# yynil/RWKVTTS

Measured on AMD Instinct MI355X. Metric: audio-tokens/sec/GPU (train fwd+bwd) RWKV7-0.4B L=4096; 1->8 GPU scaling, higher is better.
Workload: dtype bf16; 1 GPU; RWKV7-0.4B Spark layout train step (fwd+bwd+AdamW), B=8/GPU L=4096, synthetic text+speech tokens, random init (BASELINE.json configs[1]); global_batch=8, seq_len=4096, parallelism=dp1, grad_allreduce=none

## Files before the change

### include/rwkv7_hip.h

```cpp
#ifndef RWKV7_HIP_H
#define RWKV7_HIP_H

#include <stddef.h>

#ifdef __cplusplus
extern "C" {
#endif

#define RWKV7_OK 0
#define RWKV7_EINVAL (-1)
#define RWKV7_ECHUNK (-2)
#define RWKV7_EHEAD  (-3)
#define RWKV7_ESHAPE (-4)

#define RWKV7_HEAD_SIZE 64
#define RWKV7_CHUNK_LEN 16

typedef void *rwkv7_stream_t;

const char *rwkv7_version(void);

int rwkv7_wkv_fwd_bf16(int B, int T, int H, const void *w, const void *q, const void *k, const void *v,
                       const void *a, const void *b, void *y, float *s, float *sa, rwkv7_stream_t stream);
int rwkv7_wkv_fwd_f32(int B, int T, int H, const void *w, const void *q, const void *k, const void *v,
// ... 145 lines not shown
                            int nblocks, rwkv7_stream_t stream);
int rwkv7_tmix_post_bwd_compact_bf16(long rows, int D, const void *dout, const void *y, const void *r, const void *k,
                                     const void *v, const void *g, const void *gn_w, const void *gn_b, const void *r_k,
                                     float eps, void *d_y, void *dt, void *d_g, float *hscal, float *dparams_partial,
                                     int nblocks, rwkv7_stream_t stream);
int rwkv7_tmix_post_bwd_compact_f32(long rows, int D, const void *dout, const void *y, const void *r, const void *k,
                                    const void *v, const void *g, const void *gn_w, const void *gn_b, const void *r_k,
                                    float eps, void *d_y, void *dt, void *d_g, float *hscal, float *dparams_partial,
                                    int nblocks, rwkv7_stream_t stream);

int rwkv7_relusq_fwd_bf16(long n, const void *x, void *y, rwkv7_stream_t stream);
int rwkv7_relusq_fwd_f32(long n, const void *x, void *y, rwkv7_stream_t stream);
int rwkv7_relusq_bwd_bf16(long n, const void *x, const void *dy, void *dx, rwkv7_stream_t stream);
int rwkv7_relusq_bwd_f32(long n, const void *x, const void *dy, void *dx, rwkv7_stream_t stream);
int rwkv7_relusq_bwd_s_bf16(long n, const void *s, const void *dy, void *dx, rwkv7_stream_t stream);
int rwkv7_relusq_bwd_s_f32(long n, const void *s, const void *dy, void *dx, rwkv7_stream_t stream);

#define RWKV7_CHUNK_T 32
#define RWKV7_Q15_REC (64 * 64 + 2 * 256)
int rwkv7_wkv_chunk_prep_bf16(int B, int T, int H, const void *w, const void *a, const void *b, float *tinv,
                              rwkv7_stream_t stream);
int rwkv7_wkv_chunk_prep_f32(int B, int T, int H, const void *w, const void *a, const void *b, float *tinv,
                             rwkv7_stream_t stream);
int rwkv7_wkv_chunk_fwd_bf16(int B, int T, int H, const void *w, const void *q, const void *k, const void *v,
                             const void *a, const void *b, const float *tinv, void *y, float *sa, void *hs,
                             rwkv7_stream_t stream);
int rwkv7_wkv_chunk_fwd_f32(int B, int T, int H, const void *w, const void *q, const void *k, const void *v,
                            const void *a, const void *b, const float *tinv, void *y, float *sa, void *hs,
                            rwkv7_stream_t stream);
int rwkv7_wkv_chunk_fwd_seq_bf16(int B, int T, int H, const void *w, const void *q, const void *k, const void *v,
                                 const void *a, const void *b, const float *tinv, void *y, float *sa, void *hs,
                                 const int *seq_chunk_off, int nseq, rwkv7_stream_t stream);
int rwkv7_wkv_chunk_fwd_seq_f32(int B, int T, int H, const void *w, const void *q, const void *k, const void *v,
                                const void *a, const void *b, const float *tinv, void *y, float *sa, void *hs,
                                const int *seq_chunk_off, int nseq, rwkv7_stream_t stream);
int rwkv7_wkv_chunk_bseq_bf16(int B, int T, int H, const void *w, const void *q, const void *a, const void *b, const void *dy,
                              const float *tinv, void *e_vk, float *z, const int *seq_chunk_off, int nseq, rwkv7_stream_t stream);
int rwkv7_wkv_chunk_bwd_out_z_bf16(int B, int T, int H, const void *w, const void *q, const void *k, const void *v,
                                   const void *a, const void *b, const void *dy, const void *hs, const float *sa,
                                   const float *z, const void *e_vk, void *dw, void *dq, void *dk, void *dv,
                                   void *da, void *db, rwkv7_stream_t stream);
int rwkv7_wkv_chunk_fwd_state_bf16(int B, int T, int H, const void *w, const void *q, const void *k, const void *v,
                                   const void *a, const void *b, const float *tinv, void *y, float *sa, void *hs,
                                   const float *h0, float *hT, rwkv7_stream_t stream);
int rwkv7_wkv_chunk_bseq_state_bf16(int B, int T, int H, const void *w, const void *q, const void *a, const void *b,
                                    const void *dy, const float *tinv, void *e_vk, float *z,
// ... 193 lines not shown
```

### rwkvtts_amd/csrc/capi.hip

```cpp
#include <hip/hip_runtime.h>
#include <math.h>

#include "../../include/rwkv7_hip.h"

namespace rwkv7 {
int wkv_fwd_bf16(int, int, int, const void *, const void *, const void *, const void *, const void *, const void *,
                 void *, float *, float *, float *, int, hipStream_t);
int wkv_fwd_f32(int, int, int, const void *, const void *, const void *, const void *, const void *, const void *,
                void *, float *, float *, float *, int, hipStream_t);
int wkv_bwd_bf16(int, int, int, const void *, const void *, const void *, const void *, const void *, const void *,
                 const void *, const float *, const float *, void *, void *, void *, void *, void *, void *,
                 hipStream_t);
int wkv_bwd_f32(int, int, int, const void *, const void *, const void *, const void *, const void *, const void *,
                const void *, const float *, const float *, void *, void *, void *, void *, void *, void *,
                hipStream_t);

int wkv_bwd_split_bf16(int, int, int, const void *, const void *, const void *, const void *, const void *, const void *,
                       const void *, const float *, const float *, void *const *, void *const *, void *const *, void *,
                       void *const *, void *const *, int, hipStream_t);
int wkv_bwd_split_f32(int, int, int, const void *, const void *, const void *, const void *, const void *, const void *,
                      const void *, const float *, const float *, void *const *, void *const *, void *const *, void *,
                      void *const *, void *const *, int, hipStream_t);
int chunk_prep_bf16(int, int, int, const void *, const void *, const void *, float *, hipStream_t);
int chunk_prep_f32(int, int, int, const void *, const void *, const void *, float *, hipStream_t);
int chunk_fwd_bf16(int, int, int, const void *, const void *, const void *, const void *, const void *, const void *,
                   const float *, void *, float *, void *, const int *, int, hipStream_t);
int chunk_fwd_f32(int, int, int, const void *, const void *, const void *, const void *, const void *, const void *,
                  const float *, void *, float *, void *, const int *, int, hipStream_t);
int chunk_debug_mma(const float *, const float *, float *, float *, hipStream_t);
int chunk_debug_tr16(const uint16_t *, const int *, uint16_t *, hipStream_t);
int gemv32_bf16(int, int, int, const void *, const void *, const void *, void *, hipStream_t);
int ce_fwd_bwd(long, int, long, void *, const long *, long, float, float *, float, hipStream_t);
int adamw_step(long, float *, const void *, float *, float *, void *, const uint8_t *, const float *, const float *, float, float, float, float,
               float, float, float, hipStream_t);
int lora32_bf16(int, int, int, int, int, const void *, const void *, const void *, const void *, void *, hipStream_t);
int chunk_bseq_bf16(int, int, int, const void *, const void *, const void *, const void *, const void *, const float *, void *,
                    float *, const int *, int, hipStream_t);
int chunk_bseq_state_seq_bf16(int, int, int, const void *, const void *, const void *, const void *, const void *, const float *,
                              void *, float *, const int *, int, const float *, float *, hipStream_t);
int chunk_fwd9_state_seq_bf16(int, int, int, const void *, const void *, const void *, const void *, const void *, const void *,
                              const float *, void *, float *, void *, const int *, int, const float *, float *, hipStream_t);
int gemm_nt4_bf16(int, int, int, const void *, const void *, void *, const void *, int, hipStream_t);
struct MixLoraDesc {
    int nb;
    int r[4], off[4];
    int act[4];
    const void *w1[4];
// ... 393 lines not shown
                                   rwkv7_stream_t stream) {                                                         \
        if (B <= 0 || T <= 0 || H <= 0 || any_null({w, a, b, tinv})) return RWKV7_EINVAL;                           \
        if (T % RWKV7_CHUNK_T != 0) return RWKV7_ECHUNK;                                                            \
        return rwkv7::chunk_prep_##SFX(B, T, H, w, a, b, tinv, (hipStream_t)stream);                                \
    }                                                                                                               \
    int rwkv7_wkv_chunk_fwd_##SFX(int B, int T, int H, const void *w, const void *q, const void *k, const void *v,  \
                                  const void *a, const void *b, const float *tinv, void *y, float *sa, void *hs,   \
                                  rwkv7_stream_t stream) {                                                          \
        if (B <= 0 || T <= 0 || H <= 0 || any_null({w, q, k, v, a, b, tinv, y})) return RWKV7_EINVAL;               \
        if ((sa == nullptr) != (hs == nullptr)) return RWKV7_EINVAL;                                                \
        if (T % RWKV7_CHUNK_T != 0) return RWKV7_ECHUNK;                                                            \
        return rwkv7::chunk_fwd_##SFX(B, T, H, w, q, k, v, a, b, tinv, y, sa, hs, nullptr, 0, (hipStream_t)stream); \
    }                                                                                                               \
    int rwkv7_wkv_chunk_fwd_seq_##SFX(int B, int T, int H, const void *w, const void *q, const void *k, const void *v, \
                                      const void *a, const void *b, const float *tinv, void *y, float *sa, void *hs, \
                                      const int *seq_chunk_off, int nseq, rwkv7_stream_t stream) {                  \
        if (B <= 0 || T <= 0 || H <= 0 || any_null({w, q, k, v, a, b, tinv, y})) return RWKV7_EINVAL;               \
        if ((sa == nullptr) != (hs == nullptr) || (seq_chunk_off != nullptr && nseq <= 0)) return RWKV7_EINVAL;    \
        if (T % RWKV7_CHUNK_T != 0) return RWKV7_ECHUNK;                                                            \
        return rwkv7::chunk_fwd_##SFX(B, T, H, w, q, k, v, a, b, tinv, y, sa, hs, seq_chunk_off, nseq, (hipStream_t)stream); \
    }
CHUNK_DEFINE(bf16)
CHUNK_DEFINE(f32)
int rwkv7_wkv_chunk_bseq_bf16(int B, int T, int H, const void *w, const void *q, const void *a, const void *b, const void *dy,
                              const float *tinv, void *e_vk, float *z, const int *seq_chunk_off, int nseq, rwkv7_stream_t stream) {
    if (B <= 0 || T <= 0 || H <= 0 || any_null({w, q, a, b, dy, (const void *)tinv, (const void *)e_vk})) return RWKV7_EINVAL;
    if (seq_chunk_off != nullptr && nseq <= 0) return RWKV7_EINVAL;
    if (T % 32 != 0) return RWKV7_ECHUNK;
    return rwkv7::chunk_bseq_bf16(B, T, H, w, q, a, b, dy, tinv, e_vk, z, seq_chunk_off, nseq, (hipStream_t)stream);
}
int rwkv7_wkv_chunk_fwd_state_seq_bf16(int B, int T, int H, const void *w, const void *q, const void *k, const void *v,
                                       const void *a, const void *b, const float *tinv, void *y, float *sa, void *hs,
                                       const int *seq_chunk_off, int nseq, const float *h0, float *hT, rwkv7_stream_t stream) {
    if (B <= 0 || T <= 0 || H <= 0 || any_null({w, q, k, v, a, b, (const void *)tinv, y})) return RWKV7_EINVAL;
    if ((sa == nullptr) != (hs == nullptr)) return RWKV7_EINVAL;
    if ((seq_chunk_off == nullptr) != (nseq <= 0)) return RWKV7_EINVAL;
    if (T % 32 != 0) return RWKV7_ECHUNK;
    return rwkv7::chunk_fwd9_state_seq_bf16(B, T, H, w, q, k, v, a, b, tinv, y, sa, hs, seq_chunk_off, nseq, h0, hT, (hipStream_t)stream);
}
int rwkv7_wkv_chunk_bseq_state_seq_bf16(int B, int T, int H, const void *w, const void *q, const void *a, const void *b,
                                        const void *dy, const float *tinv, void *e_vk, float *z, const int *seq_chunk_off, int nseq,
                                        const float *dhT, float *dh0, rwkv7_stream_t stream) {
    if (B <= 0 || T <= 0 || H <= 0 || any_null({w, q, a, b, dy, (const void *)tinv, (const void *)e_vk})) return RWKV7_EINVAL;
    if ((seq_chunk_off == nullptr) != (nseq <= 0)) return RWKV7_EINVAL;
    if (T % 32 != 0) return RWKV7_ECHUNK;
    return rwkv7::chunk_bseq_state_seq_bf16(B, T, H, w, q, a, b, dy, tinv, e_vk, z, seq_chunk_off, nseq, dhT, dh0, (hipStream_t)stream);
// ... 399 lines not shown
```

### rwkvtts_amd/csrc/elementwise.hip

```cpp
#include "ln_row.h"

namespace rwkv7 {

__device__ __forceinline__ float sigmoidf_(float x) { return 1.0f / (1.0f + __expf(-x)); }

template <typename T, int NMIX>
__global__ __launch_bounds__(kEwMaxThreads) void mix_fwd_kernel(int B, int T_, int D, const T *__restrict__ x, const T *__restrict__ x_prev,
                               const T *__restrict__ mask, const T *__restrict__ params, T *__restrict__ out) {
    const int c = threadIdx.x * 8;
    const long rows = (long)B * T_;
    float p[NMIX][8];
#pragma unroll
    for (int i = 0; i < NMIX; i++) V8<T>::ld(params + (long)i * D + c, p[i]);
    const bool has_mask = mask != nullptr;
    const T *const maskq = has_mask ? mask : params;
    for (long row = blockIdx.x; row < rows; row += gridDim.x) {
        const int t = (int)(row % T_);
        const long rp = row > 0 ? row - 1 : 0;
        Raw8<T> qc, qp;
        qc.load(x + row * D + c);
        qp.load(x + rp * D + c);
        const float mc0 = V8<T>::ld1(maskq + (has_mask ? row : 0)), mp0 = V8<T>::ld1(maskq + (has_mask ? rp : 0));
        float xc[8], xp[8];
        qc.get(xc);
        qp.get(xp);
        const float mc = has_mask ? mc0 : 1.f, mp = (has_mask ? mp0 : 1.f) * (t > 0 ? 1.f : 0.f);
#pragma unroll
// ... 93 lines not shown
            for (int i = 0; i < NMIX; i++) {
                float gc[8];
                A.g[i].get(gc);
#pragma unroll
                for (int j = 0; j < 8; j++) {
                    acc[j] = fmaf(gc[j], 1.f - p[i][j], acc[j]);
                    acc[j] = fmaf(gn[i][j], p[i][j], acc[j]);
                    dp[i][j] = fmaf(gc[j], xp[j] - xc[j], dp[i][j]);
                    gn[i][j] = gc[j] * first;
                }
            }
#pragma unroll
            for (int j = 0; j < 8; j++) {
                acc[j] *= m;
                xc[j] = xq[j];
            }
            V8<T>::st(dx + row * D + c, acc);
            A = Bn;
        }
    }
#pragma unroll
    for (int i = 0; i < NMIX; i++) V8<float>::st(dpart + ((long)blockIdx.x * NMIX + i) * D + c, dp[i]);
}

__device__ __forceinline__ float softplus_(float u) { return u > 20.f ? u : log1pf(__expf(u)); }

template <typename T>
__global__ __launch_bounds__(kEwMaxThreads) void tmix_prepare_fwd_kernel(long rows, int D, const T *__restrict__ w_pre, const T *__restrict__ k,
                                        const T *__restrict__ v, const T *__restrict__ a_pre,
                                        const T *__restrict__ v_pre, const T *__restrict__ v_first,
                                        const T *__restrict__ mask, const T *__restrict__ k_k,
                                        const T *__restrict__ k_a, T *__restrict__ w_out, T *__restrict__ k_out,
                                        T *__restrict__ v_out, T *__restrict__ a_out, T *__restrict__ b_out) {
    const int c = threadIdx.x * 8;
    float kk_p[8], ka_p[8];
    V8<T>::ld(k_k + c, kk_p);
    V8<T>::ld(k_a + c, ka_p);
    for (long row = blockIdx.x; row < rows; row += gridDim.x) {
        const long o = row * D + c;
        const float m = mask ? V8<T>::ld1(mask + row) : 1.f;
        float z[8], kx[8], vx[8], ap[8];
        V8<T>::ld(w_pre + o, z);
        V8<T>::ld(k + o, kx);
        V8<T>::ld(v + o, vx);
        V8<T>::ld(a_pre + o, ap);
        float wo[8], ko[8], vo[8], ao[8], bo[8], kkr[8];
        float ss = 0.f;
#pragma unroll
        for (int j = 0; j < 8; j++) {
            wo[j] = (-softplus_(-z[j]) - 0.5f) * m;
            kx[j] *= m;
            vx[j] *= m;
            kkr[j] = kx[j] * kk_p[j];
            ss = fmaf(kkr[j], kkr[j], ss);
        }
        if (v_pre) {
            float vp[8], vf[8];
            V8<T>::ld(v_pre + o, vp);
            V8<T>::ld(v_first + o, vf);
#pragma unroll
            for (int j = 0; j < 8; j++) vx[j] = fmaf(vf[j] - vx[j], sigmoidf_(vp[j]), vx[j]);
        }
        ss = sum8(ss);
        const float inv = m / fmaxf(sqrtf(ss), 1e-12f);
#pragma unroll
        for (int j = 0; j < 8; j++) {
            const float a = sigmoidf_(ap[j]);
            const float kk = kkr[j] * inv;
            ko[j] = kx[j] * fmaf(a - 1.f, ka_p[j], 1.f);
            vo[j] = vx[j] * m;
            ao[j] = -kk;
            bo[j] = kk * a;
        }
        V8<T>::st(w_out + o, wo);
        V8<T>::st(k_out + o, ko);
        V8<T>::st(v_out + o, vo);
        V8<T>::st(a_out + o, ao);
        V8<T>::st(b_out + o, bo);
    }
}

template <typename T>
struct PrepBwdExtra {
    const T *d_w_b, *d_k2_b, *d_k2_c, *d_v2_b, *d_a_b, *d_b_b;
    const T *d_r_a, *d_r_b, *d_r_c;
    T *d_r;
    const T *d_vfirst_in;
    const T *dt, *r, *r_k;
    const float *hscal;
};

template <typename T, bool MULTI>
__global__ __launch_bounds__(kEwMaxThreads) void tmix_prepare_bwd_kernel(long rows, int D, const T *__restrict__ w_pre, const T *__restrict__ k,
                                        const T *__restrict__ v, const T *__restrict__ a_pre,
                                        const T *__restrict__ v_pre, const T *__restrict__ v_first,
                                        const T *__restrict__ mask, const T *__restrict__ k_k,
// ... 1302 lines not shown
```

### rwkvtts_amd/csrc/ln_row.h

```cpp
#pragma once
#include "wkv7_common.h"

namespace rwkv7 {

constexpr int kEwMaxThreads = 512;

typedef __bf16 pkbf2_t __attribute__((ext_vector_type(2)));
typedef float pkf2_t __attribute__((ext_vector_type(2)));
__device__ __forceinline__ uint32_t pk_bf16(float a, float b) {
    const pkf2_t v = {a, b};
    return __builtin_bit_cast(uint32_t, __builtin_convertvector(v, pkbf2_t));
}

template <typename T>
struct V8;
template <>
struct V8<bf16_t> {
    static __device__ __forceinline__ void ld(const bf16_t *p, float (&f)[8]) {
        const uint4 r = *reinterpret_cast<const uint4 *>(p);
        f[0] = __uint_as_float(r.x << 16); f[1] = __uint_as_float(r.x & 0xffff0000u);
        f[2] = __uint_as_float(r.y << 16); f[3] = __uint_as_float(r.y & 0xffff0000u);
        f[4] = __uint_as_float(r.z << 16); f[5] = __uint_as_float(r.z & 0xffff0000u);
        f[6] = __uint_as_float(r.w << 16); f[7] = __uint_as_float(r.w & 0xffff0000u);
    }
    static __device__ __forceinline__ void st(bf16_t *p, const float (&f)[8]) {
        uint4 r;
        r.x = pk_bf16(f[0], f[1]);
        r.y = pk_bf16(f[2], f[3]);
        r.z = pk_bf16(f[4], f[5]);
        r.w = pk_bf16(f[6], f[7]);
        *reinterpret_cast<uint4 *>(p) = r;
    }
    static __device__ __forceinline__ float ld1(const bf16_t *p) { return bf2f(p->x); }
};
template <>
struct V8<float> {
    static __device__ __forceinline__ void ld(const float *p, float (&f)[8]) {
        const float4 a = *reinterpret_cast<const float4 *>(p), b = *reinterpret_cast<const float4 *>(p + 4);
        f[0] = a.x; f[1] = a.y; f[2] = a.z; f[3] = a.w; f[4] = b.x; f[5] = b.y; f[6] = b.z; f[7] = b.w;
    }
    static __device__ __forceinline__ void st(float *p, const float (&f)[8]) {
        *reinterpret_cast<float4 *>(p) = make_float4(f[0], f[1], f[2], f[3]);
        *reinterpret_cast<float4 *>(p + 4) = make_float4(f[4], f[5], f[6], f[7]);
    }
    static __device__ __forceinline__ float ld1(const float *p) { return *p; }
};

template <typename T>
struct Raw8;
template <>
struct Raw8<bf16_t> {
    uint4 r;
    __device__ __forceinline__ void load(const bf16_t *p) { r = *reinterpret_cast<const uint4 *>(p); }
    __device__ __forceinline__ void get(float (&f)[8]) const {
        f[0] = __uint_as_float(r.x << 16); f[1] = __uint_as_float(r.x & 0xffff0000u);
// ... 76 lines not shown
#pragma unroll
    for (int j = 0; j < 8; j++) s += v[j];
    block_sum2(s, dummy, red, ph, ng);
    ph ^= 2;
    mu = s * inv_d;
    float q = 0.f;
    dummy = 0.f;
#pragma unroll
    for (int j = 0; j < 8; j++) {
        v[j] -= mu;
        q = fmaf(v[j], v[j], q);
    }
    block_sum2(q, dummy, red, ph, ng);
    ph ^= 2;
    rs = rsqrtf(q * inv_d + eps);
    const float m = has_mask ? f.m : 1.f;
#pragma unroll
    for (int j = 0; j < 8; j++) hm[j] = round_to<T>(fmaf(v[j] * rs, gm[j], bt[j]));
    if (write && h_out) V8<T>::st(h_out + o, hm);
#pragma unroll
    for (int j = 0; j < 8; j++) hm[j] *= m;
}

}
```

### rwkvtts_amd/csrc/wkv7_chunk_fwd.hip

```cpp
#include "chunk_common.h"
#include "launch_attr.h"

namespace rwkv7 {

#ifdef WKV7C_TIMING
__device__ long long g_chunk_timing[4 * 16];
#define TSTAMP(i)                                                                  \
    do {                                                                           \
        const long long now_ = __builtin_readcyclecounter();                       \
        if (blockIdx.x == 0 && lane == 0) g_chunk_timing[wave * 16 + (i)] += now_ - tprev_; \
        tprev_ = now_;                                                             \
    } while (0)
#else
#define TSTAMP(i) do { } while (0)
#endif

template <typename T>
__device__ __forceinline__ float ld_scalar(const T *p);
template <>
__device__ __forceinline__ float ld_scalar<bf16_t>(const bf16_t *p) { return bf2f(p->x); }
template <>
__device__ __forceinline__ float ld_scalar<float>(const float *p) { return *p; }

template <typename T>
__global__ __launch_bounds__(64) __attribute__((amdgpu_waves_per_eu(4, 4))) void wkv7c_prep_kernel(int T_, int H, const T *__restrict__ w_, const T *__restrict__ a_,
                                                        const T *__restrict__ b_, float *__restrict__ tinv_) {
    constexpr int LD = kC + kPad;
    __shared__ __attribute__((aligned(16))) uint16_t planes[4 * kC * LD];
    uint16_t *ATh = planes, *ATl = planes + kC * LD, *BHh = planes + 2 * kC * LD, *BHl = planes + 3 * kC * LD;
    static_assert(2 * kC * LD * 2 >= kC * 2 * 16 * 4, "the back substitution's A^T copy must fit over the a~ planes");
    const int nc = T_ / kC;
    const int bh = blockIdx.x / nc, c = blockIdx.x - bh * nc;
    const int bb = bh / H, hh = bh - bb * H;
    const int lane = threadIdx.x;
    const int kc = lane & 31, th = lane >> 5;
    const long tstride = (long)H * kN;
    const long base = (((long)bb * T_ + (long)c * kC + 16 * th) * H + hh) * kN + kc;
    float wv[2][16], av_[2][16], bv_[2][16];
#pragma unroll
    for (int p = 0; p < 2; p++)
#pragma unroll
        for (int j = 0; j < 16; j++) {
            const long idx = base + 32 * p + j * tstride;
            wv[p][j] = ld_scalar<T>(w_ + idx);
            av_[p][j] = ld_scalar<T>(a_ + idx);
            bv_[p][j] = ld_scalar<T>(b_ + idx);
        }
    f32x16 acc = zero16();
#pragma unroll
    for (int p = 0; p < 2; p++) {
        float lw[16], tot = 0.f;
#pragma unroll
        for (int j = 0; j < 16; j++) {
            lw[j] = -fast_exp(wv[p][j]);
            tot += lw[j];
        }
        const float first = __shfl(tot, kc);
        float G = th ? first : 0.f;
        if (p == 1) __syncthreads();
#pragma unroll
        for (int j = 0; j < 16; j++) {
            const int t = 16 * th + j;
            const float at = av_[p][j] * fast_exp(G);
            G += lw[j];
            const float bh_ = bv_[p][j] * fast_exp(-G);
            split2(at, ATh[t * LD + kc], ATl[t * LD + kc]);
            split2(bh_, BHh[t * LD + kc], BHl[t * LD + kc]);
        }
        __syncthreads();
        mma_tile3<kC>(acc, BHh, BHl, LD, ATh, ATl, LD, lane);
// ... 342 lines not shown
    for (int i = lane; i < kC * kC; i += 64) DT[i] = bf2f(Oh[(i / kC) * LDC + i % kC]) + bf2f(Ol[(i / kC) * LDC + i % kC]);
}

typedef short v4s_t __attribute__((ext_vector_type(4)));
__global__ __launch_bounds__(64) void tr16_probe_kernel(const uint16_t *__restrict__ in, const int *__restrict__ addr,
                                                        uint16_t *__restrict__ out) {
    __shared__ __attribute__((aligned(16))) uint16_t sm[4096];
    for (int i = threadIdx.x; i < 4096; i += 64) sm[i] = in[i];
    __syncthreads();
    const int lane = threadIdx.x;
    const v4s_t r = __builtin_amdgcn_ds_read_tr16_b64_v4i16((v4s_t __attribute__((address_space(3))) *)(sm + addr[lane]));
#pragma unroll
    for (int j = 0; j < 4; j++) out[lane * 4 + j] = (uint16_t)r[j];
}
int chunk_debug_tr16(const uint16_t *in, const int *addr, uint16_t *out, hipStream_t st) {
    (void)hipGetLastError();
    hipLaunchKernelGGL(tr16_probe_kernel, dim3(1), dim3(64), 0, st, in, addr, out);
    return (int)hipGetLastError();
}

template <typename T>
static int launch_prep(int B, int T_, int H, const void *w, const void *a, const void *b, float *tinv, hipStream_t st) {
    (void)hipGetLastError();
    hipLaunchKernelGGL((wkv7c_prep_kernel<T>), dim3(B * H * (T_ / kC)), dim3(64), 0, st, T_, H, (const T *)w, (const T *)a,
                       (const T *)b, tinv);
    return (int)hipGetLastError();
}

template <typename T, bool SAVE>
static int launch_fwd_t(int B, int T_, int H, const void *w, const void *q, const void *k, const void *v, const void *a,
                        const void *b, const float *tinv, void *y, float *sa, void *hs, const int *seq_off, int nseq,
                        hipStream_t st) {
    static DynLdsOnce lds_once;
    if (hipError_t e = lds_once.ensure(reinterpret_cast<const void *>(&wkv7c_fwd_kernel<T, SAVE>), (int)FwdSmem::total<T>()); e != hipSuccess) return (int)e;
    (void)hipGetLastError();
    hipLaunchKernelGGL((wkv7c_fwd_kernel<T, SAVE>), dim3((seq_off ? nseq : B) * H * 2), dim3(256), FwdSmem::total<T>(), st, T_, H,
                       (const T *)w, (const T *)q, (const T *)k, (const T *)v, (const T *)a, (const T *)b, tinv, (T *)y, sa, (uint16_t *)hs, seq_off);
    return (int)hipGetLastError();
}

int chunk_prep_bf16(int B, int T_, int H, const void *w, const void *a, const void *b, float *tinv, hipStream_t st) {
    return launch_prep<bf16_t>(B, T_, H, w, a, b, tinv, st);
}
int chunk_prep_f32(int B, int T_, int H, const void *w, const void *a, const void *b, float *tinv, hipStream_t st) {
    return launch_prep<float>(B, T_, H, w, a, b, tinv, st);
}
int chunk_fwd9_bf16(int, int, int, const void *, const void *, const void *, const void *, const void *, const void *, const float *,
                    void *, float *, void *, const int *, int, hipStream_t);

int chunk_fwd_bf16(int B, int T_, int H, const void *w, const void *q, const void *k, const void *v, const void *a,
                   const void *b, const float *tinv, void *y, float *sa, void *hs, const int *seq_off, int nseq, hipStream_t st) {
    return chunk_fwd9_bf16(B, T_, H, w, q, k, v, a, b, tinv, y, sa, hs, seq_off, nseq, st);
}
#ifdef RWKV7_LAB
int chunk_fwd4_bf16(int B, int T_, int H, const void *w, const void *q, const void *k, const void *v, const void *a,
                    const void *b, const float *tinv, void *y, float *sa, void *hs, const int *seq_off, int nseq, hipStream_t st) {
    return (sa && hs) ? launch_fwd_t<bf16_t, true>(B, T_, H, w, q, k, v, a, b, tinv, y, sa, hs, seq_off, nseq, st)
                      : launch_fwd_t<bf16_t, false>(B, T_, H, w, q, k, v, a, b, tinv, y, nullptr, nullptr, seq_off, nseq, st);
}
#endif
int chunk_fwd_f32(int B, int T_, int H, const void *w, const void *q, const void *k, const void *v, const void *a,
                  const void *b, const float *tinv, void *y, float *sa, void *hs, const int *seq_off, int nseq, hipStream_t st) {
    return (sa && hs) ? launch_fwd_t<float, true>(B, T_, H, w, q, k, v, a, b, tinv, y, sa, hs, seq_off, nseq, st)
// ... 20 lines not shown
```

### rwkvtts_amd/fused.py

```python
import ctypes
import os

import torch

from . import _lib

_FWD_BLOCKS = 32768
_MIX_FWD_BLOCKS = 2048
_BWD_BLOCKS = 1024
_MIX_BWD_ROWS = 4
_MIX_BWD_BLOCKS = 1024


def _p(t):
    return None if t is None else ctypes.c_void_p(t.data_ptr())


def _stream(t):
    return ctypes.c_void_p(torch.cuda.current_stream(t.device).cuda_stream)


def _sfx(t):
    if not t.is_cuda:
        raise NotImplementedError("fused RWKV-7 stages run on the HIP device only (no CPU path)")
# ... 539 lines not shown
        y, r, k, v, g, gn_w, gn_b, r_k = ctx.saved_tensors
        B, T, D = y.shape
        rows = B * T
        nb = min(rows, _BWD_BLOCKS)
        dout = _c(dout)
        d_y, d_r, d_k, d_v, d_g = [torch.empty_like(y) for _ in range(5)]
        part = torch.empty(nb, 3, D, dtype=torch.float32, device=y.device)
        _call("tmix_post_bwd", y, ctypes.c_long(rows), D, _p(dout), _p(y), _p(r), _p(k), _p(v), _p(g), _p(gn_w), _p(gn_b), _p(r_k),
              ctypes.c_float(ctx.eps), _p(d_y), _p(d_r), _p(d_k), _p(d_v), _p(d_g), _p(part), nb)
        dp = _colsum(part, y.dtype)
        return d_y, d_r, d_k, d_v, d_g, dp[0], dp[1], dp[2], None


def tmix_post(y, r, k, v, g, gn_weight, gn_bias, r_k, H, eps):
    return _TmixPost.apply(y, r, k, v, g, gn_weight, gn_bias, r_k.reshape(-1), eps)


CHAIN_VFIRST_GRAD = True
CHUNKED_WKV_BWD = True
CHUNKED_WKV_FWD = True
VIA_REFERENCE_OP = False


class _TmixCore(torch.autograd.Function):

    @staticmethod
    def forward(ctx, r, w_pre, k, v, a_pre, g, v_pre, v_first, k_k, k_a, gn_w, gn_b, r_k, mask, H, eps, seq_start=None):
        from . import ops
        B, T, D = k.shape
        if T % ops.CHUNK_LEN != 0:
            raise ValueError(f"T={T} must be a multiple of {ops.CHUNK_LEN}")
        r, w_pre, k, v, a_pre, g = _c(r), _c(w_pre), _c(k), _c(v), _c(a_pre), _c(g)
        v_pre = None if v_pre is None else _c(v_pre)
        v_first = None if v_first is None else _c(v_first)
        k_k, k_a = _c(k_k.to(k.dtype)), _c(k_a.to(k.dtype))
        gn_w, gn_b, r_k = _c(gn_w.to(k.dtype)), _c(gn_b.to(k.dtype)), _c(r_k.reshape(-1).to(k.dtype))
        rows = B * T
        w, k2, v2, a_in, b_in = [torch.empty_like(k) for _ in range(5)]
        _call("tmix_prepare_fwd", k, ctypes.c_long(rows), D, _p(w_pre), _p(k), _p(v), _p(a_pre), _p(v_pre), _p(v_first),
              _p(mask), _p(k_k), _p(k_a), _p(w), _p(k2), _p(v2), _p(a_in), _p(b_in), min(rows, _FWD_BLOCKS))
        v4 = lambda t: t.view(B, T, H, 64)
        via_op = VIA_REFERENCE_OP and seq_start is None
        chunked = CHUNKED_WKV_FWD and CHUNKED_WKV_BWD and k.dtype == torch.bfloat16 and T % ops.CHUNK_T == 0 and not via_op
        if seq_start is not None and not chunked:
            raise ValueError("packed rows (seq_start) need the chunked WKV7 kernels: bf16 tensors, T % 32 == 0")
        if chunked:
            y4, tinv, sa, s = ops.wkv7_chunk_forward(v4(w), v4(r), v4(k2), v4(v2), v4(a_in), v4(b_in), seq_off=seq_start)
            y = y4.view(B, T, D)
        else:
            tinv = None
            y = torch.empty_like(k)
            s = torch.empty(B, H, T // ops.CHUNK_LEN, 64, 64, dtype=torch.float32, device=k.device)
            sa = torch.empty(B, T, H, 64, dtype=torch.float32, device=k.device)
            if via_op:
                torch.ops.wind_backstepping.forward(v4(w), v4(r), v4(k2), v4(v2), v4(a_in), v4(b_in), v4(y), s, sa)
            else:
                ops.wkv7_forward_scalar(v4(w), v4(r), v4(k2), v4(v2), v4(a_in), v4(b_in), v4(y), s, sa)
        out = torch.empty_like(k)
        _call("tmix_post_fwd", k, ctypes.c_long(rows), D, _p(y), _p(r), _p(k2), _p(v2), _p(g), _p(gn_w), _p(gn_b), _p(r_k),
              ctypes.c_float(eps), _p(out), min(rows, _FWD_BLOCKS))
        ctx.save_for_backward(r, w_pre, k, v, a_pre, g, v_pre, v_first, k_k, k_a, gn_w, gn_b, r_k, mask,
                              w, k2, v2, a_in, b_in, y, s, sa, tinv)
        ctx.H, ctx.eps, ctx.chunked_fwd, ctx.seq_start, ctx.via_op = H, eps, chunked, seq_start, via_op
        ctx.set_materialize_grads(False)
        if v_first is None or not CHAIN_VFIRST_GRAD:
            return out
        return out, v_first.view_as(v_first)

    @staticmethod
    def backward(ctx, dout, d_vf_next=None):
# ... 604 lines not shown
```

### rwkvtts_amd/ops.py

```python
import ctypes

import torch

from . import _lib, fused

HEAD_SIZE = 64
CHUNK_LEN = 16
DTYPE = torch.bfloat16


KERNEL_TIMERS = None


class _timed:
    def __init__(self, name, ref):
        self.name, self.on = name, KERNEL_TIMERS is not None
        if self.on:
            st = torch.cuda.current_stream(ref.device)
            self.s, self.e, self.st = torch.cuda.Event(enable_timing=True), torch.cuda.Event(enable_timing=True), st

    def __enter__(self):
        if self.on:
            self.s.record(self.st)

# ... 225 lines not shown
    q = rec[..., :4096].float().index_select(-1, mi)
    sc = rec[..., 4096:].contiguous().view(torch.float32).index_select(-1, si)
    return (q * sc).reshape(*rec.shape[:-1], 64, 64)


def wkv7_chunk_prep(w, a, b):
    B, T, H, C = w.shape
    sfx = _sfx([w, a, b], "wkv7_chunk_prep")
    tinv = torch.empty(B, H, T // CHUNK_T, CHUNK_T, CHUNK_T, dtype=torch.float32, device=w.device)
    with torch.cuda.device_of(w), _timed("wkv7c_prep", w):
        rc = getattr(_lib.lib(), "rwkv7_wkv_chunk_prep_" + sfx)(B, T, H, _p(w), _p(a), _p(b), _p(tinv), _stream(w))
    _lib.check(rc, "wkv7_chunk_prep")
    return tinv


def _nseq(seq_off):
    if seq_off is None:
        return 0
    if seq_off.dtype != torch.int32 or seq_off.dim() != 1 or seq_off.numel() < 2 or not seq_off.is_contiguous() or not seq_off.is_cuda:
        raise TypeError("seq_off must be a contiguous int32 [nseq + 1] device tensor")
    return seq_off.numel() - 1


def _chunk_fwd(w, q, k, v, a, b, save, seq_off, nseq, h0=None):
    B, T, H, C = w.shape
    sfx = _sfx([w, q, k, v, a, b], "wkv7_chunk_forward")
    if T % CHUNK_T != 0:
        raise ValueError(f"chunked WKV7 needs T % {CHUNK_T} == 0, got T={T}")
    tinv = wkv7_chunk_prep(w, a, b)
    y = torch.empty_like(v)
    sa = torch.empty(B, T, H, C, dtype=torch.float32, device=w.device) if save else None
    hs = torch.empty(B, H, T // CHUNK_T, Q15_REC, dtype=torch.int16, device=w.device) if save else None
    hT = None if h0 is None else torch.empty(nseq if seq_off is not None else B, H, C, C, dtype=torch.float32, device=w.device)
    args = (B, T, H, _p(w), _p(q), _p(k), _p(v), _p(a), _p(b), _p(tinv), _p(y), _p(sa), _p(hs), _p(seq_off), nseq)
    with torch.cuda.device_of(w), _timed("wkv7c_fwd" if h0 is None else "wkv7c_fwd_state", w):
        if h0 is None:
            rc = getattr(_lib.lib(), "rwkv7_wkv_chunk_fwd_seq_" + sfx)(*args, _stream(w))
        else:
            rc = _lib.lib().rwkv7_wkv_chunk_fwd_state_seq_bf16(*args, _p(h0), _p(hT), _stream(w))
    _lib.check(rc, "wkv7_chunk_forward")
    return y, tinv, sa, hs, hT


def wkv7_chunk_forward(w, q, k, v, a, b, save=True, seq_off=None):
    y, tinv, sa, hs, _ = _chunk_fwd(w, q, k, v, a, b, save, seq_off, _nseq(seq_off))
    return (y, tinv, sa, hs) if save else y


def _bseq(w, q, a, b, dy, tinv, seq_off, nseq, want_z, state=None):
    B, T, H, C = w.shape
    if w.dtype != torch.bfloat16:
        raise TypeError("the chunked backward is bf16 only")
    if T % CHUNK_T != 0:
        raise ValueError(f"chunked WKV7 needs T % {CHUNK_T} == 0, got T={T}")
    e_vk = torch.empty(B, H, T // CHUNK_T, Q15_REC, dtype=torch.int16, device=w.device)
    zeroed = seq_off is not None and state is None
    z = (torch.zeros if zeroed else torch.empty)(B, T, H, C, dtype=torch.float32, device=w.device) if want_z else None
    args = (B, T, H, _p(w), _p(q), _p(a), _p(b), _p(dy), _p(tinv), _p(e_vk), _p(z), _p(seq_off), nseq)
    with torch.cuda.device_of(w), _timed("wkv7c_bseq" if state is None else "wkv7c_bseq_state", w):
        if state is None:
            rc = _lib.lib().rwkv7_wkv_chunk_bseq_bf16(*args, _stream(w))
        else:
            rc = _lib.lib().rwkv7_wkv_chunk_bseq_state_seq_bf16(*args, *[_p(t) for t in state], _stream(w))
    _lib.check(rc, "wkv7_chunk_bseq")
    return e_vk, z


def wkv7_chunk_bwd_seq(w, q, a, b, dy, tinv, seq_off=None, want_z=False):
# ... 183 lines not shown
```

Before: 279,400 tokens/s.

## Fuse time-mix prepare elementwise stage into the WKV7 chunk prep kernel

Adds a variant of the chunk-prep (tinv) kernel that computes the tmix prepare elementwise math (w, k2, v2, a, b) itself, writes those outputs, and stages w, a and b through shared memory to build the chunk inverse. This removes one separate elementwise launch and the global re-read of w, a and b by the prep kernel. The forward then reuses the precomputed tinv. In exchange the prep kernel does more work per 64-thread block with a different access pattern, uses extra LDS round trips with barriers, and may lose the occupancy the standalone elementwise kernel had. The path is on by default through an environment flag.

```diff
diff --git a/include/rwkv7_hip.h b/include/rwkv7_hip.h
--- a/include/rwkv7_hip.h
+++ b/include/rwkv7_hip.h
@@ -191,6 +191,9 @@
                               rwkv7_stream_t stream);
 int rwkv7_wkv_chunk_prep_f32(int B, int T, int H, const void *w, const void *a, const void *b, float *tinv,
                              rwkv7_stream_t stream);
+int rwkv7_tmix_prepare_prep_bf16(int B, int T, int D, const void *w_pre, const void *k, const void *v, const void *a_pre,
+                                 const void *v_pre, const void *v_first, const void *mask, const void *k_k, const void *k_a, void *w,
+                                 void *k2, void *v2, void *ain, void *bin, float *tinv, rwkv7_stream_t stream);
 int rwkv7_wkv_chunk_fwd_bf16(int B, int T, int H, const void *w, const void *q, const void *k, const void *v,
                              const void *a, const void *b, const float *tinv, void *y, float *sa, void *hs,
                              rwkv7_stream_t stream);
diff --git a/rwkvtts_amd/csrc/capi.hip b/rwkvtts_amd/csrc/capi.hip
--- a/rwkvtts_amd/csrc/capi.hip
+++ b/rwkvtts_amd/csrc/capi.hip
@@ -23,6 +23,8 @@
                       void *const *, void *const *, int, hipStream_t);
 int chunk_prep_bf16(int, int, int, const void *, const void *, const void *, float *, hipStream_t);
 int chunk_prep_f32(int, int, int, const void *, const void *, const void *, float *, hipStream_t);
+int chunk_prepare_prep_bf16(int, int, int, const void *, const void *, const void *, const void *, const void *, const void *, const void *,
+                            const void *, const void *, void *, void *, void *, void *, void *, float *, hipStream_t);
 int chunk_fwd_bf16(int, int, int, const void *, const void *, const void *, const void *, const void *, const void *,
                    const float *, void *, float *, void *, const int *, int, hipStream_t);
 int chunk_fwd_f32(int, int, int, const void *, const void *, const void *, const void *, const void *, const void *,
@@ -462,6 +464,20 @@
     }
 CHUNK_DEFINE(bf16)
 CHUNK_DEFINE(f32)
+int rwkv7_tmix_prepare_prep_bf16(int B, int T, int D, const void *w_pre, const void *k, const void *v, const void *a_pre,
+                                 const void *v_pre, const void *v_first, const void *mask, const void *k_k, const void *k_a, void *w,
+                                 void *k2, void *v2, void *ain, void *bin, float *tinv, rwkv7_stream_t stream) {
+    if (B <= 0 || T <= 0 || D <= 0 || any_null({w_pre, k, v, a_pre, k_k, k_a, (const void *)w, (const void *)k2, (const void *)v2,
+                                                (const void *)ain, (const void *)bin, (const void *)tinv}))
+        return RWKV7_EINVAL;
+    if ((v_pre == nullptr) != (v_first == nullptr)) return RWKV7_EINVAL;
+    if (T % RWKV7_CHUNK_T != 0) return RWKV7_ECHUNK;
+    if (D % RWKV7_HEAD_SIZE != 0) return RWKV7_ESHAPE;
+    const int H = D / RWKV7_HEAD_SIZE;
+    if ((long)B * H * (T / RWKV7_CHUNK_T) > 0x7fffffffL) return RWKV7_ESHAPE;
+    return rwkv7::chunk_prepare_prep_bf16(B, T, H, w_pre, k, v, a_pre, v_pre, v_first, mask, k_k, k_a, w, k2, v2, ain, bin, tinv,
+                                          (hipStream_t)stream);
+}
 int rwkv7_wkv_chunk_bseq_bf16(int B, int T, int H, const void *w, const void *q, const void *a, const void *b, const void *dy,
                               const float *tinv, void *e_vk, float *z, const int *seq_chunk_off, int nseq, rwkv7_stream_t stream) {
     if (B <= 0 || T <= 0 || H <= 0 || any_null({w, q, a, b, dy, (const void *)tinv, (const void *)e_vk})) return RWKV7_EINVAL;
diff --git a/rwkvtts_amd/csrc/elementwise.hip b/rwkvtts_amd/csrc/elementwise.hip
--- a/rwkvtts_amd/csrc/elementwise.hip
+++ b/rwkvtts_amd/csrc/elementwise.hip
@@ -1,8 +1,6 @@
 #include "ln_row.h"
 
 namespace rwkv7 {
-
-__device__ __forceinline__ float sigmoidf_(float x) { return 1.0f / (1.0f + __expf(-x)); }
 
 template <typename T, int NMIX>
 __global__ __launch_bounds__(kEwMaxThreads) void mix_fwd_kernel(int B, int T_, int D, const T *__restrict__ x, const T *__restrict__ x_prev,
@@ -142,8 +140,6 @@
 #pragma unroll
     for (int i = 0; i < NMIX; i++) V8<float>::st(dpart + ((long)blockIdx.x * NMIX + i) * D + c, dp[i]);
 }
-
-__device__ __forceinline__ float softplus_(float u) { return u > 20.f ? u : log1pf(__expf(u)); }
 
 template <typename T>
 __global__ __launch_bounds__(kEwMaxThreads) void tmix_prepare_fwd_kernel(long rows, int D, const T *__restrict__ w_pre, const T *__restrict__ k,
@@ -165,33 +161,15 @@
         V8<T>::ld(v + o, vx);
         V8<T>::ld(a_pre + o, ap);
         float wo[8], ko[8], vo[8], ao[8], bo[8], kkr[8];
-        float ss = 0.f;
-#pragma unroll
-        for (int j = 0; j < 8; j++) {
-            wo[j] = (-softplus_(-z[j]) - 0.5f) * m;
-            kx[j] *= m;
-            vx[j] *= m;
-            kkr[j] = kx[j] * kk_p[j];
-            ss = fmaf(kkr[j], kkr[j], ss);
-        }
+        float ss = prepare_row_head(z, kx, vx, m, kk_p, wo, kkr);
         if (v_pre) {
             float vp[8], vf[8];
             V8<T>::ld(v_pre + o, vp);
             V8<T>::ld(v_first + o, vf);
-#pragma unroll
-            for (int j = 0; j < 8; j++) vx[j] = fmaf(vf[j] - vx[j], sigmoidf_(vp[j]), vx[j]);
+            prepare_row_vres(vx, vp, vf);
         }
         ss = sum8(ss);
-        const float inv = m / fmaxf(sqrtf(ss), 1e-12f);
-#pragma unroll
-        for (int j = 0; j < 8; j++) {
-            const float a = sigmoidf_(ap[j]);
-            const float kk = kkr[j] * inv;
-            ko[j] = kx[j] * fmaf(a - 1.f, ka_p[j], 1.f);
-            vo[j] = vx[j] * m;
-            ao[j] = -kk;
-            bo[j] = kk * a;
-        }
+        prepare_row_tail(ss, m, ap, kx, vx, kkr, ka_p, ko, vo, ao, bo);
         V8<T>::st(w_out + o, wo);
         V8<T>::st(k_out + o, ko);
         V8<T>::st(v_out + o, vo);
diff --git a/rwkvtts_amd/csrc/ln_row.h b/rwkvtts_amd/csrc/ln_row.h
--- a/rwkvtts_amd/csrc/ln_row.h
+++ b/rwkvtts_amd/csrc/ln_row.h
@@ -23,14 +23,15 @@
         f[4] = __uint_as_float(r.z << 16); f[5] = __uint_as_float(r.z & 0xffff0000u);
         f[6] = __uint_as_float(r.w << 16); f[7] = __uint_as_float(r.w & 0xffff0000u);
     }
-    static __device__ __forceinline__ void st(bf16_t *p, const float (&f)[8]) {
+    static __device__ __forceinline__ uint4 pack(const float (&f)[8]) {
         uint4 r;
         r.x = pk_bf16(f[0], f[1]);
         r.y = pk_bf16(f[2], f[3]);
         r.z = pk_bf16(f[4], f[5]);
         r.w = pk_bf16(f[6], f[7]);
-        *reinterpret_cast<uint4 *>(p) = r;
+        return r;
     }
+    static __device__ __forceinline__ void st(bf16_t *p, const float (&f)[8]) { *reinterpret_cast<uint4 *>(p) = pack(f); }
     static __device__ __forceinline__ float ld1(const bf16_t *p) { return bf2f(p->x); }
 };
 template <>
@@ -153,4 +154,39 @@
     for (int j = 0; j < 8; j++) hm[j] *= m;
 }
 
+__device__ __forceinline__ float sigmoidf_(float x) { return 1.0f / (1.0f + __expf(-x)); }
+__device__ __forceinline__ float softplus_(float u) { return u > 20.f ? u : log1pf(__expf(u)); }
+
+__device__ __forceinline__ float prepare_row_head(const float (&z)[8], float (&kx)[8], float (&vx)[8], float m, const float (&kk_p)[8],
+                                                  float (&wo)[8], float (&kkr)[8]) {
+    float ss = 0.f;
+#pragma unroll
+    for (int j = 0; j < 8; j++) {
+        wo[j] = (-softplus_(-z[j]) - 0.5f) * m;
+        kx[j] *= m;
+        vx[j] *= m;
+        kkr[j] = kx[j] * kk_p[j];
+        ss = fmaf(kkr[j], kkr[j], ss);
+    }
+    return ss;
 }
+__device__ __forceinline__ void prepare_row_vres(float (&vx)[8], const float (&vp)[8], const float (&vf)[8]) {
+#pragma unroll
+    for (int j = 0; j < 8; j++) vx[j] = fmaf(vf[j] - vx[j], sigmoidf_(vp[j]), vx[j]);
+}
+__device__ __forceinline__ void prepare_row_tail(float ss, float m, const float (&ap)[8], const float (&kx)[8], const float (&vx)[8],
+                                                 const float (&kkr)[8], const float (&ka_p)[8], float (&ko)[8], float (&vo)[8],
+                                                 float (&ao)[8], float (&bo)[8]) {
+    const float inv = m / fmaxf(sqrtf(ss), 1e-12f);
+#pragma unroll
+    for (int j = 0; j < 8; j++) {
+        const float a = sigmoidf_(ap[j]);
+        const float kk = kkr[j] * inv;
+        ko[j] = kx[j] * fmaf(a - 1.f, ka_p[j], 1.f);
+        vo[j] = vx[j] * m;
+        ao[j] = -kk;
+        bo[j] = kk * a;
+    }
+}
+
+}
diff --git a/rwkvtts_amd/csrc/wkv7_chunk_fwd.hip b/rwkvtts_amd/csrc/wkv7_chunk_fwd.hip
--- a/rwkvtts_amd/csrc/wkv7_chunk_fwd.hip
+++ b/rwkvtts_amd/csrc/wkv7_chunk_fwd.hip
@@ -1,5 +1,6 @@
 #include "chunk_common.h"
 #include "launch_attr.h"
+#include "ln_row.h"
 
 namespace rwkv7 {
 
@@ -22,9 +23,14 @@
 template <>
 __device__ __forceinline__ float ld_scalar<float>(const float *p) { return *p; }
 
-template <typename T>
+struct PrepareIo {
+    const bf16_t *w_pre, *k, *v, *a_pre, *v_pre, *v_first, *mask, *k_k, *k_a;
+    bf16_t *w, *k2, *v2, *ain, *bin;
+};
+
+template <typename T, int PREPARE>
 __global__ __launch_bounds__(64) __attribute__((amdgpu_waves_per_eu(4, 4))) void wkv7c_prep_kernel(int T_, int H, const T *__restrict__ w_, const T *__restrict__ a_,
-                                                        const T *__restrict__ b_, float *__restrict__ tinv_) {
+                                                        const T *__restrict__ b_, float *__restrict__ tinv_, PrepareIo io) {
     constexpr int LD = kC + kPad;
     __shared__ __attribute__((aligned(16))) uint16_t planes[4 * kC * LD];
     uint16_t *ATh = planes, *ATl = planes + kC * LD, *BHh = planes + 2 * kC * LD, *BHl = planes + 3 * kC * LD;
@@ -37,15 +43,105 @@
     const long tstride = (long)H * kN;
     const long base = (((long)bb * T_ + (long)c * kC + 16 * th) * H + hh) * kN + kc;
     float wv[2][16], av_[2][16], bv_[2][16];
-#pragma unroll
-    for (int p = 0; p < 2; p++)
-#pragma unroll
-        for (int j = 0; j < 16; j++) {
-            const long idx = base + 32 * p + j * tstride;
-            wv[p][j] = ld_scalar<T>(w_ + idx);
-            av_[p][j] = ld_scalar<T>(a_ + idx);
-            bv_[p][j] = ld_scalar<T>(b_ + idx);
-        }
+    if constexpr (PREPARE == 0) {
+#pragma unroll
+        for (int p = 0; p < 2; p++)
+#pragma unroll
+            for (int j = 0; j < 16; j++) {
+                const long idx = base + 32 * p + j * tstride;
+                wv[p][j] = ld_scalar<T>(w_ + idx);
+                av_[p][j] = ld_scalar<T>(a_ + idx);
+                bv_[p][j] = ld_scalar<T>(b_ + idx);
+            }
+    } else {
+        static_assert(PREPARE == 0 || sizeof(T) == 2, "the prepare stage in front of the inverse is bf16 only");
+        constexpr int kStage = (kC + 1) * kN;
+        static_assert(2 * kStage <= 4 * kC * LD, "w and a staging rows must fit over the operand planes");
+        const int rg = lane >> 3, cg = lane & 7;
+        const long D = (long)H * kN;
+        const long row0 = (long)bb * T_ + (long)c * kC + rg;
+        const int col = hh * kN + cg * 8;
+        float kk_p[8], ka_p[8];
+        V8<bf16_t>::ld(io.k_k + col, kk_p);
+        V8<bf16_t>::ld(io.k_a + col, ka_p);
+        const bool has_mask = io.mask != nullptr;
+        const bf16_t *const maskq = has_mask ? io.mask : io.k_k;
+        struct Pre {
+            Raw8<bf16_t> z, kx, vx, ap, vp, vf;
+            float m;
+        };
+        auto fetch = [&](int g) {
+            Pre f;
+            const long row = row0 + 8 * g, o = row * D + col;
+            f.z.load(io.w_pre + o);
+            f.kx.load(io.k + o);
+            f.vx.load(io.v + o);
+            f.ap.load(io.a_pre + o);
+            if (PREPARE == 2) {
+                f.vp.load(io.v_pre + o);
+                f.vf.load(io.v_first + o);
+            }
+            f.m = V8<bf16_t>::ld1(maskq + (has_mask ? row : 0));
+            return f;
+        };
+        uint4 bq[4];
+        auto stage = [&](int slot, int g, uint4 q) {
+            const int t = 8 * g + rg;
+            *reinterpret_cast<uint4 *>(planes + slot * kStage + (t + (t >> 4)) * kN + cg * 8) = q;
+        };
+        auto row_group = [&](int g, const Pre &f) {
+            const long o = (row0 + 8 * g) * D + col;
+            const float m = has_mask ? f.m : 1.f;
+            float z[8], kx[8], vx[8], ap[8];
+            f.z.get(z);
+            f.kx.get(kx);
+            f.vx.get(vx);
+            f.ap.get(ap);
+            float wo[8], ko[8], vo[8], ao[8], bo[8], kkr[8];
+            float ss = prepare_row_head(z, kx, vx, m, kk_p, wo, kkr);
+            if (PREPARE == 2) {
+                float vp[8], vf[8];
+                f.vp.get(vp);
+                f.vf.get(vf);
+                prepare_row_vres(vx, vp, vf);
+            }
+            ss = sum8(ss);
+            prepare_row_tail(ss, m, ap, kx, vx, kkr, ka_p, ko, vo, ao, bo);
+            const uint4 wq = V8<bf16_t>::pack(wo), aq = V8<bf16_t>::pack(ao);
+            bq[g] = V8<bf16_t>::pack(bo);
+            *reinterpret_cast<uint4 *>(io.w + o) = wq;
+            V8<bf16_t>::st(io.k2 + o, ko);
+            V8<bf16_t>::st(io.v2 + o, vo);
+            *reinterpret_cast<uint4 *>(io.ain + o) = aq;
+            *reinterpret_cast<uint4 *>(io.bin + o) = bq[g];
+            stage(0, g, wq);
+            stage(1, g, aq);
+        };
+        {
+            Pre f0 = fetch(0), f1 = fetch(1);
+            row_group(0, f0);
+            f0 = fetch(2);
+            row_group(1, f1);
+            f1 = fetch(3);
+            row_group(2, f0);
+            row_group(3, f1);
+        }
+        auto unstage = [&](int slot, float (&x)[2][16]) {
+#pragma unroll
+            for (int p = 0; p < 2; p++)
+#pragma unroll
+                for (int j = 0; j < 16; j++) x[p][j] = bf2f(planes[slot * kStage + (16 * th + j + th) * kN + 32 * p + kc]);
+        };
+        __syncthreads();
+        unstage(0, wv);
+        unstage(1, av_);
+        __syncthreads();
+#pragma unroll
+        for (int g = 0; g < 4; g++) stage(0, g, bq[g]);
+        __syncthreads();
+        unstage(0, bv_);
+        __syncthreads();
+    }
     f32x16 acc = zero16();
 #pragma unroll
     for (int p = 0; p < 2; p++) {
@@ -434,8 +530,8 @@
 template <typename T>
 static int launch_prep(int B, int T_, int H, const void *w, const void *a, const void *b, float *tinv, hipStream_t st) {
     (void)hipGetLastError();
-    hipLaunchKernelGGL((wkv7c_prep_kernel<T>), dim3(B * H * (T_ / kC)), dim3(64), 0, st, T_, H, (const T *)w, (const T *)a,
-                       (const T *)b, tinv);
+    hipLaunchKernelGGL((wkv7c_prep_kernel<T, 0>), dim3(B * H * (T_ / kC)), dim3(64), 0, st, T_, H, (const T *)w, (const T *)a,
+                       (const T *)b, tinv, PrepareIo{});
     return (int)hipGetLastError();
 }
 
@@ -451,6 +547,21 @@
     return (int)hipGetLastError();
 }
 
+int chunk_prepare_prep_bf16(int B, int T_, int H, const void *w_pre, const void *k, const void *v, const void *a_pre, const void *v_pre,
+                            const void *v_first, const void *mask, const void *k_k, const void *k_a, void *w, void *k2, void *v2,
+                            void *ain, void *bin, float *tinv, hipStream_t st) {
+    using P = const bf16_t *;
+    using Q = bf16_t *;
+    const PrepareIo io{(P)w_pre, (P)k, (P)v, (P)a_pre, (P)v_pre, (P)v_first, (P)mask, (P)k_k, (P)k_a, (Q)w, (Q)k2, (Q)v2, (Q)ain, (Q)bin};
+    const dim3 grid(B * H * (T_ / kC)), block(64);
+    const P none = nullptr;
+    (void)hipGetLastError();
+    if (v_pre)
+        hipLaunchKernelGGL((wkv7c_prep_kernel<bf16_t, 2>), grid, block, 0, st, T_, H, none, none, none, tinv, io);
+    else
+        hipLaunchKernelGGL((wkv7c_prep_kernel<bf16_t, 1>), grid, block, 0, st, T_, H, none, none, none, tinv, io);
+    return (int)hipGetLastError();
+}
 int chunk_prep_bf16(int B, int T_, int H, const void *w, const void *a, const void *b, float *tinv, hipStream_t st) {
     return launch_prep<bf16_t>(B, T_, H, w, a, b, tinv, st);
 }
diff --git a/rwkvtts_amd/fused.py b/rwkvtts_amd/fused.py
--- a/rwkvtts_amd/fused.py
+++ b/rwkvtts_amd/fused.py
@@ -585,6 +585,23 @@
 VIA_REFERENCE_OP = False
 
 
+PREPARE_PREP = os.environ.get("RWKV7_PREPARE_PREP", "1") == "1"
+
+
+def tmix_prepare_prep(w_pre, k, v, a_pre, v_pre, v_first, mask, k_k, k_a):
+    from . import ops
+    B, T, D = k.shape
+    if k.dtype != torch.bfloat16 or T % ops.CHUNK_T != 0 or D % 64 != 0:
+        raise ValueError(f"tmix_prepare_prep: bf16, T % {ops.CHUNK_T} == 0 and D % 64 == 0 expected, got {k.dtype} {tuple(k.shape)}")
+    w, k2, v2, a_in, b_in = [torch.empty_like(k) for _ in range(5)]
+    tinv = torch.empty(B, D // 64, T // ops.CHUNK_T, ops.CHUNK_T, ops.CHUNK_T, dtype=torch.float32, device=k.device)
+    with torch.cuda.device_of(k), ops._timed("wkv7c_prep", k):
+        rc = _lib.lib().rwkv7_tmix_prepare_prep_bf16(B, T, D, _p(w_pre), _p(k), _p(v), _p(a_pre), _p(v_pre), _p(v_first), _p(mask),
+                                                     _p(k_k), _p(k_a), _p(w), _p(k2), _p(v2), _p(a_in), _p(b_in), _p(tinv), _stream(k))
+    _lib.check(rc, "tmix_prepare_prep")
+    return w, k2, v2, a_in, b_in, tinv
+
+
 class _TmixCore(torch.autograd.Function):
 
     @staticmethod
@@ -599,16 +616,20 @@
         k_k, k_a = _c(k_k.to(k.dtype)), _c(k_a.to(k.dtype))
         gn_w, gn_b, r_k = _c(gn_w.to(k.dtype)), _c(gn_b.to(k.dtype)), _c(r_k.reshape(-1).to(k.dtype))
         rows = B * T
-        w, k2, v2, a_in, b_in = [torch.empty_like(k) for _ in range(5)]
-        _call("tmix_prepare_fwd", k, ctypes.c_long(rows), D, _p(w_pre), _p(k), _p(v), _p(a_pre), _p(v_pre), _p(v_first),
-              _p(mask), _p(k_k), _p(k_a), _p(w), _p(k2), _p(v2), _p(a_in), _p(b_in), min(rows, _FWD_BLOCKS))
         v4 = lambda t: t.view(B, T, H, 64)
         via_op = VIA_REFERENCE_OP and seq_start is None
         chunked = CHUNKED_WKV_FWD and CHUNKED_WKV_BWD and k.dtype == torch.bfloat16 and T % ops.CHUNK_T == 0 and not via_op
         if seq_start is not None and not chunked:
             raise ValueError("packed rows (seq_start) need the chunked WKV7 kernels: bf16 tensors, T % 32 == 0")
+        tinv = None
+        if chunked and PREPARE_PREP:
+            w, k2, v2, a_in, b_in, tinv = tmix_prepare_prep(w_pre, k, v, a_pre, v_pre, v_first, mask, k_k, k_a)
+        else:
+            w, k2, v2, a_in, b_in = [torch.empty_like(k) for _ in range(5)]
+            _call("tmix_prepare_fwd", k, ctypes.c_long(rows), D, _p(w_pre), _p(k), _p(v), _p(a_pre), _p(v_pre), _p(v_first),
+                  _p(mask), _p(k_k), _p(k_a), _p(w), _p(k2), _p(v2), _p(a_in), _p(b_in), min(rows, _FWD_BLOCKS))
         if chunked:
-            y4, tinv, sa, s = ops.wkv7_chunk_forward(v4(w), v4(r), v4(k2), v4(v2), v4(a_in), v4(b_in), seq_off=seq_start)
+            y4, tinv, sa, s = ops.wkv7_chunk_forward(v4(w), v4(r), v4(k2), v4(v2), v4(a_in), v4(b_in), seq_off=seq_start, tinv=tinv)
             y = y4.view(B, T, D)
         else:
             tinv = None
diff --git a/rwkvtts_amd/ops.py b/rwkvtts_amd/ops.py
--- a/rwkvtts_amd/ops.py
+++ b/rwkvtts_amd/ops.py
@@ -271,12 +271,15 @@
     return seq_off.numel() - 1
 
 
-def _chunk_fwd(w, q, k, v, a, b, save, seq_off, nseq, h0=None):
+def _chunk_fwd(w, q, k, v, a, b, save, seq_off, nseq, h0=None, tinv=None):
     B, T, H, C = w.shape
     sfx = _sfx([w, q, k, v, a, b], "wkv7_chunk_forward")
     if T % CHUNK_T != 0:
         raise ValueError(f"chunked WKV7 needs T % {CHUNK_T} == 0, got T={T}")
-    tinv = wkv7_chunk_prep(w, a, b)
+    if tinv is None:
+        tinv = wkv7_chunk_prep(w, a, b)
+    elif tinv.dtype != torch.float32 or tuple(tinv.shape) != (B, H, T // CHUNK_T, CHUNK_T, CHUNK_T) or not tinv.is_contiguous():
+        raise TypeError(f"wkv7_chunk_forward: tinv must be contiguous float32 {(B, H, T // CHUNK_T, CHUNK_T, CHUNK_T)}")
     y = torch.empty_like(v)
     sa = torch.empty(B, T, H, C, dtype=torch.float32, device=w.device) if save else None
     hs = torch.empty(B, H, T // CHUNK_T, Q15_REC, dtype=torch.int16, device=w.device) if save else None
@@ -291,8 +294,8 @@
     return y, tinv, sa, hs, hT
 
 
-def wkv7_chunk_forward(w, q, k, v, a, b, save=True, seq_off=None):
-    y, tinv, sa, hs, _ = _chunk_fwd(w, q, k, v, a, b, save, seq_off, _nseq(seq_off))
+def wkv7_chunk_forward(w, q, k, v, a, b, save=True, seq_off=None, tinv=None):
+    y, tinv, sa, hs, _ = _chunk_fwd(w, q, k, v, a, b, save, seq_off, _nseq(seq_off), tinv=tinv)
     return (y, tinv, sa, hs) if save else y
 
 
```

Result: no change. 280,800 tokens/s (median of 6 runs) (+0.5%).
